# KyanChen/RSPrompter

Measured on NVIDIA H100. Metric: images/sec, higher is better.
Workload: dtype bf16

## Files before the change

### include/rsp_b200.h

```cpp
#ifndef RSP_B200_H_
#define RSP_B200_H_

#include <stdint.h>

#ifdef __cplusplus
extern "C" {
#endif

#define RSP_ABI_VERSION 2

int rsp_abi_version(void);
const char* rsp_last_error(void);

int rsp_gemm_bf16(const void* A, int lda, const void* W, int ldw, void* out, int ldo, int M, int N,
                  int K, const float* bias, const void* residual, int ldr, int res_fp32, int res_mod,
                  const int32_t* row_map, int act, int out_fp32, void* stream);

int rsp_conv3x3_nhwc_bf16(const void* x, int B, int H, int W, int C, const void* Wt, int ldw, void* out, int ldo,
                          int N, const float* bias, const void* residual, int ldr, int res_fp32, int act,
                          int out_fp32, void* stream);
int rsp_conv3x3_geometry_ok(int B, int H, int W, int C);

int rsp_gemm_bf16_simt(const void* A, int lda, const void* W, int ldw, void* out, int ldo, int M,
                       int N, int K, const float* bias, const void* residual, int ldr, int res_fp32,
                       int res_mod, const int32_t* row_map, int act, int out_fp32, void* stream);

int rsp_vit_attention(const void* qkv, const void* rel_h, const void* rel_w, void* out, int n_seq,
                      int T, int S, int H, int hd, void* stream);
int rsp_vit_attention_scatter(const void* qkv, const void* rel_h, const void* rel_w, void* out, int n_seq, int T,
                              int Sg, int H, int hd, const int32_t* out_row_map, void* stream);

int rsp_vit_attention_simt(const void* qkv, const void* rel_h, const void* rel_w, void* out,
                           int n_seq, int T, int S, int H, int hd, void* stream);

int rsp_layernorm(const void* in, int in_fp32, int ld_in, void* out, int out_fp32, int ld_out,
                  const float* gamma, const float* beta, const int32_t* src_map, int rows_out, int C,
                  float eps, int act, void* copy_out, int ld_copy, void* stream);

int rsp_layernorm_add(const void* x, const void* res, int res_fp32, const int32_t* res_block_map,
                      int res_block_rows, const float* gamma, const float* beta, void* out, const float* pos,
                      int pos_mod, void* out_pe, long long rows, int C, float eps, void* stream);

int rsp_patchify16(const float* img, void* out, int B, int H, int W, void* stream);

int rsp_im2col_nhwc(const void* in, void* out, int B, int H, int W, int C, int KH, int KW,
                    int stride, int pad, void* stream);

int rsp_nhwc_to_nchw(const void* in, int in_fp32, float* out, int B, int HW, int C, void* stream);

int rsp_gemm_bf16_ex(const void* A, int lda, const void* W, int ldw, void* out, int ldo, int M, int N,
                     int K, const float* bias, const void* residual, int ldr, int res_fp32, int res_mod,
                     const int32_t* row_map, int act, int out_fp32, int epi_mode, const float* ln_gamma,
                     const float* ln_beta, float ln_eps, const int32_t* res_block_map,
// ... 158 lines not shown
                         int64_t* offsets, void* stream);
int rsp_mask_rle_write(const uint8_t* src, int packed, const int64_t* desc, int n, const int64_t* offsets, char* pool,
                       int32_t* lengths, void* stream);
int rsp_mask_rle_placed_lengths(const uint8_t* src, int packed, const int64_t* desc, const int64_t* desc_host, int n,
                                int64_t* offsets, void* stream);
int rsp_mask_rle_placed_write(const uint8_t* src, int packed, const int64_t* desc, int n, const int64_t* offsets,
                              char* pool, int32_t* lengths, void* stream);


int rsp_preprocess_u8(const uint8_t* img, int h, int w, long long stride_c, long long stride_y, long long stride_x,
                      float* out, int H, int W, const float* mean3, const float* std3, int swap_rb, float pad_value,
                      void* stream);

int rsp_resize_pad_u8(const int64_t* desc, const int64_t* desc_host, int B, float* out, int Hp, int Wp,
                      const float* mean3, const float* std3, int swap_rb, const float* pad3, void* stream);

int rsp_patchify16_u8(const uint8_t* img, int hwc, void* out, int B, int H, int W, const float* mean3, const float* std3,
                      int swap_rb, void* stream);

int rsp_cast_f32_bf16(const float* in, void* out, long long n, void* stream);

int rsp_add_table_bf16(const void* x, const float* table, void* out, long long n, long long period, void* stream);

#ifdef __cplusplus
}
#endif
#endif
```

### rsprompter_b200/_lib.py

```python
from __future__ import annotations

import ctypes
import os
import subprocess
from pathlib import Path

import torch

_PKG_DIR = Path(__file__).resolve().parent
LIB_PATH = _PKG_DIR / "librsp_b200.so"
CSRC_DIR = _PKG_DIR / "csrc"


class RspError(RuntimeError):
    """Raised when an ``rsp_*`` entry point returns a non-zero status."""


def build_library(verbose: bool = False) -> Path:
    cmd = ["make", "-C", str(CSRC_DIR), "-j", str(os.cpu_count() or 4), "all"]
    res = subprocess.run(cmd, capture_output=True, text=True)
    if res.returncode != 0:
        raise RuntimeError(f"building librsp_b200.so failed:\n{res.stdout[-4000:]}\n{res.stderr[-4000:]}")
    if verbose:
        print(res.stdout[-2000:])
    return LIB_PATH


def _load() -> ctypes.CDLL:
    if not LIB_PATH.exists():
        raise ImportError(
            f"{LIB_PATH} not found: the CUDA extension is mandatory (no fallback path). "
            "Run `python -c 'import __graft_entry__ as g; g.build()'` or `make -C rsprompter_b200/csrc`.")
    return ctypes.CDLL(str(LIB_PATH))


_lib = _load()

_vp, _i, _f = ctypes.c_void_p, ctypes.c_int, ctypes.c_float

_SIGNATURES = {
    "rsp_abi_version": ([], _i),
    "rsp_last_error": ([], ctypes.c_char_p),
    "rsp_gemm_bf16": ([_vp, _i, _vp, _i, _vp, _i, _i, _i, _i, _vp, _vp, _i, _i, _i, _vp, _i, _i, _vp], _i),
    "rsp_gemm_bf16_simt": ([_vp, _i, _vp, _i, _vp, _i, _i, _i, _i, _vp, _vp, _i, _i, _i, _vp, _i, _i, _vp], _i),
    "rsp_vit_attention": ([_vp, _vp, _vp, _vp, _i, _i, _i, _i, _i, _vp], _i),
    "rsp_vit_attention_scatter": ([_vp, _vp, _vp, _vp, _i, _i, _i, _i, _i, _vp, _vp], _i),
    "rsp_vit_attention_simt": ([_vp, _vp, _vp, _vp, _i, _i, _i, _i, _i, _vp], _i),
    "rsp_layernorm": ([_vp, _i, _i, _vp, _i, _i, _vp, _vp, _vp, _i, _i, _f, _i, _vp, _i, _vp], _i),
    "rsp_patchify16": ([_vp, _vp, _i, _i, _i, _vp], _i),
    "rsp_layernorm_add": ([_vp, _vp, _i, _vp, _i, _vp, _vp, _vp, _vp, _i, _vp, ctypes.c_longlong, _i, _f, _vp], _i),
    "rsp_im2col_nhwc": ([_vp, _vp, _i, _i, _i, _i, _i, _i, _i, _i, _vp], _i),
    "rsp_nhwc_to_nchw": ([_vp, _i, _vp, _i, _i, _i, _vp], _i),
    "rsp_cast_f32_bf16": ([_vp, _vp, ctypes.c_longlong, _vp], _i),
    "rsp_add_table_bf16": ([_vp, _vp, _vp, ctypes.c_longlong, ctypes.c_longlong, _vp], _i),
    "rsp_gemm_bf16_ex": ([_vp, _i, _vp, _i, _vp, _i, _i, _i, _i, _vp, _vp, _i, _i, _i, _vp, _i, _i,
                          _i, _vp, _vp, _f, _vp, _i, _vp, _vp, _i, _i, _vp], _i),
    "rsp_add_cast_bf16": ([_vp, _vp, _vp, ctypes.c_longlong, ctypes.c_longlong, _vp], _i),
    "rsp_token_self_attention": ([_vp, _vp, _vp, _vp, _i, _i, _i, _i, _vp], _i),
    "rsp_t2i_attention": ([_vp, _vp, _vp, _i, _vp, _vp, _i, _i, _i, _vp], _i),
    "rsp_i2t_attention": ([_vp, _vp, _vp, _vp, _vp, _i, _i, _i, _vp], _i),
    "rsp_t2i_fused": ([_vp, _i, _vp, _vp, _vp, _vp, _vp, _i, _i, _i, _vp], _i),
    "rsp_i2t_fused": ([_vp, _i, _vp, _vp, _vp, _vp, _vp, _vp, _vp, _vp, _vp, _f, _vp, _i, _i, _i, _vp], _i),
    "rsp_rpn_decode": ([_vp, _i, _vp, _i, _i, _i, _i, _i, _i, _vp, _vp, _f, _f, _f, _i, _i, _vp, _vp, _vp], _i),
    "rsp_bbox_cls_decode": ([_vp, _i, _vp, _i, _vp, _vp, _i, _i, _vp, _f, _f, _f, _vp, _vp, _vp, _vp], _i),
    "rsp_rpn_decode_shapes": ([_vp, _i, _vp, _i, _i, _i, _i, _i, _i, _vp, _vp, _vp, _f, _i, _i, _vp, _vp, _vp], _i),
    "rsp_nms_batched_topk": ([_vp, _vp, _vp, _i, _i, _f, _vp, _vp, _vp, _i, _vp], _i),
    "rsp_bbox_cls_decode_shapes": ([_vp, _i, _vp, _i, _vp, _vp, _i, _i, _vp, _vp, _f, _vp, _vp, _vp, _vp], _i),
    "rsp_nms_batched": ([_vp, _vp, _vp, _i, _i, _f, _vp, _vp, _vp, _vp], _i),
    "rsp_compact_keep": ([_vp, _vp, _vp, _vp, _i, _i, _i, _vp, _vp, _vp, _vp, _vp, _vp], _i),
    "rsp_soft_nms_workspace_bytes": ([_i, _i, _i, _vp], _i),
    "rsp_soft_nms_batched": ([_vp, _vp, _vp, _vp, _i, _i, _i, _f, _f, _f, _i, _i, _i, _vp, ctypes.c_size_t, _vp, _vp,
                              _vp, _vp, _vp, _vp], _i),
    "rsp_roi_align_nhwc": ([_vp, _vp, _vp, _vp, _vp, _i, _vp, _i, _i, _i, _f, _vp, _vp], _i),
    "rsp_mask_paste": ([_vp, _vp, _i, _i, _i, _i, _i, _f, _i, _vp], _i),
    "rsp_pool2_nhwc": ([_vp, _vp, _i, _i, _i, _i, _i, _vp], _i),
    "rsp_zero_border_nhwc": ([_vp, _i, _i, _i, _i, _vp], _i),
    "rsp_sigmoid_f32": ([_vp, _vp, ctypes.c_longlong, _vp], _i),
# ... 336 lines not shown


def i2t_attention(Q: torch.Tensor, ktok: torch.Tensor, vtok: torch.Tensor, hw: int,
                  q_block: torch.Tensor | None = None) -> torch.Tensor:
    global launch_count
    _require_cuda(Q, ktok, vtok, q_block)
    N, Tq, C = ktok.shape
    assert C == 128 and Q.dtype == torch.bfloat16 and Q.is_contiguous() and Q.shape[1] == 128
    assert ktok.dtype == torch.bfloat16 and vtok.dtype == torch.bfloat16
    assert ktok.is_contiguous() and vtok.is_contiguous() and vtok.shape == ktok.shape
    if q_block is not None:
        assert q_block.dtype == torch.int32 and q_block.numel() == N and q_block.is_contiguous()
    else:
        assert Q.shape[0] == N * hw
    out = torch.empty((N * hw, 128), device=Q.device, dtype=torch.bfloat16)
    _check(_lib.rsp_i2t_attention(_ptr(Q), _ptr(q_block), _ptr(ktok), _ptr(vtok), _ptr(out), N, Tq, hw, _stream()),
           "rsp_i2t_attention")
    launch_count += 1
    return out


def vit_attention(qkv: torch.Tensor, rel_h: torch.Tensor, rel_w: torch.Tensor, n_seq: int, S: int,
                  H: int, hd: int, *, out: torch.Tensor | None = None, simt: bool = False,
                  out_row_map: torch.Tensor | None = None, out_rows: int | None = None) -> torch.Tensor:
    global launch_count
    _require_cuda(qkv, rel_h, rel_w, out)
    T = S * S
    D = H * hd
    if not simt and out_row_map is None and S not in (14, 32, 64) and T % 128 == 0 and S % 4 == 0:
        return vit_attention_generic(qkv, rel_h, rel_w, n_seq, S, H, hd, out=out)
    if not simt and S in (14, 32, 64):
        _log("attention_window" if S == 14 else "attention_global", 4.0 * n_seq * H * T * T * hd)
    assert qkv.dtype == torch.bfloat16 and qkv.is_contiguous() and qkv.shape == (n_seq * T, 3 * D)
    assert rel_h.dtype == torch.bfloat16 and rel_h.is_contiguous() and rel_h.shape == (2 * S - 1, hd)
    assert rel_w.dtype == torch.bfloat16 and rel_w.is_contiguous() and rel_w.shape == (2 * S - 1, hd)
    if out_row_map is not None:
        assert not simt and out_row_map.dtype == torch.int32 and out_row_map.is_contiguous()
        assert out_row_map.numel() == n_seq * T and out_rows is not None
        _require_cuda(out_row_map)
        if out is None:
            out = torch.empty((out_rows, D), device=qkv.device, dtype=torch.bfloat16)
        assert out.dtype == torch.bfloat16 and out.is_contiguous() and out.shape == (out_rows, D)
        _check(_lib.rsp_vit_attention_scatter(_ptr(qkv), _ptr(rel_h), _ptr(rel_w), _ptr(out), n_seq, T, S, H, hd,
                                              _ptr(out_row_map), _stream()), "rsp_vit_attention_scatter")
        launch_count += 1
        return out
    if out is None:
        out = torch.empty((n_seq * T, D), device=qkv.device, dtype=torch.bfloat16)
    assert out.dtype == torch.bfloat16 and out.is_contiguous() and out.shape == (n_seq * T, D)
    fn = _lib.rsp_vit_attention_simt if simt else _lib.rsp_vit_attention
    _check(fn(_ptr(qkv), _ptr(rel_h), _ptr(rel_w), _ptr(out), n_seq, T, S, H, hd, _stream()),
           "rsp_vit_attention")
    launch_count += 1
    return out


def gemm_grouped(a: torch.Tensor, w: torch.Tensor, out: torch.Tensor, N: int, m_group_rows: int, w_group_rows: int,
                 row_map: torch.Tensor | None = None) -> torch.Tensor:
    global launch_count
    _require_cuda(a, w, out, row_map)
    assert a.dtype == torch.bfloat16 and w.dtype == torch.bfloat16 and a.dim() == 2 and w.dim() == 2
    assert a.stride(1) == 1 and w.stride(1) == 1 and out.dim() == 2 and out.stride(1) == 1
    M, K = a.shape
    assert w.shape[1] == K and M % m_group_rows == 0 and m_group_rows % 128 == 0
    assert w.shape[0] >= (M // m_group_rows - 1) * w_group_rows + N and out.shape[1] >= N
    assert out.dtype in (torch.bfloat16, torch.float32)
    if row_map is not None:
        assert row_map.dtype == torch.int32 and row_map.numel() == M and row_map.is_contiguous()
    _check(_lib.rsp_gemm_bf16_grouped(_ptr(a), a.stride(0), _ptr(w), w.stride(0), _ptr(out), out.stride(0), M, N, K,
                                      m_group_rows, w_group_rows, _ptr(row_map), int(out.dtype == torch.float32),
                                      _stream()), "rsp_gemm_bf16_grouped")
    launch_count += 1
    _log("gemm", 2.0 * M * N * K)
    return out

# ... 835 lines not shown
```

### rsprompter_b200/csrc/abi.cu

```cuda
#include "../../include/rsp_b200.h"

#include "attention.h"
#include "gemm.h"
#include "rowops.h"

namespace rsp { const char* last_error(); }
using namespace rsp;

static inline cudaStream_t S(void* s) { return static_cast<cudaStream_t>(s); }

extern "C" {

int rsp_abi_version(void) { return RSP_ABI_VERSION; }
const char* rsp_last_error(void) { return rsp::last_error(); }

static GemmArgs make_gemm_args(const void* A, int lda, const void* W, int ldw, void* out, int ldo,
                               int M, int N, int K, const float* bias, const void* residual, int ldr,
                               int res_fp32, int res_mod, const int32_t* row_map, int act,
                               int out_fp32) {
  GemmArgs a;
  a.A = A; a.lda = lda; a.W = W; a.ldw = ldw; a.out = out; a.ldo = ldo;
  a.M = M; a.N = N; a.K = K; a.bias = bias; a.residual = residual; a.ldr = ldr;
  a.res_fp32 = res_fp32; a.res_mod = res_mod; a.row_map = row_map; a.act = act;
  a.out_fp32 = out_fp32;
// ... 30 lines not shown
                       int res_mod, const int32_t* row_map, int act, int out_fp32, void* stream) {
  return gemm_bf16_simt(make_gemm_args(A, lda, W, ldw, out, ldo, M, N, K, bias, residual, ldr,
                                       res_fp32, res_mod, row_map, act, out_fp32), S(stream));
}

static AttentionArgs make_att_args(const void* qkv, const void* rel_h, const void* rel_w, void* out,
                                   int n_seq, int T, int Sg, int H, int hd, const int32_t* out_row_map = nullptr) {
  AttentionArgs a;
  a.qkv = qkv; a.rel_h = rel_h; a.rel_w = rel_w; a.out = out;
  a.n_seq = n_seq; a.T = T; a.S = Sg; a.H = H; a.hd = hd; a.out_row_map = out_row_map;
  return a;
}

int rsp_vit_attention(const void* qkv, const void* rel_h, const void* rel_w, void* out, int n_seq,
                      int T, int Sg, int H, int hd, void* stream) {
  return vit_attention(make_att_args(qkv, rel_h, rel_w, out, n_seq, T, Sg, H, hd), S(stream));
}

int rsp_vit_attention_scatter(const void* qkv, const void* rel_h, const void* rel_w, void* out, int n_seq, int T,
                              int Sg, int H, int hd, const int32_t* out_row_map, void* stream) {
  return vit_attention(make_att_args(qkv, rel_h, rel_w, out, n_seq, T, Sg, H, hd, out_row_map), S(stream));
}

int rsp_vit_attention_simt(const void* qkv, const void* rel_h, const void* rel_w, void* out,
                           int n_seq, int T, int Sg, int H, int hd, void* stream) {
  return vit_attention_simt(make_att_args(qkv, rel_h, rel_w, out, n_seq, T, Sg, H, hd), S(stream));
}

int rsp_attn_softmax_bias(const float* scores, int lds, const float* tab, int ldt, int NT, void* P, int ldp, int n_rows,
                          int T, int Sg, float scale, void* stream) {
  return attn_softmax_bias(scores, lds, tab, ldt, NT, P, ldp, n_rows, T, Sg, scale, S(stream));
}

int rsp_transpose_cols(const void* in, int ld, int col0, int C, int n_seq, int T, void* out, void* stream) {
  return transpose_cols(in, ld, col0, C, n_seq, T, out, S(stream));
}

int rsp_split_heads(const void* in, int ld, int col0, int H, int hd, int n_seq, int T, void* out, void* stream) {
  return split_heads(in, ld, col0, H, hd, n_seq, T, out, S(stream));
}

int rsp_layernorm(const void* in, int in_fp32, int ld_in, void* out, int out_fp32, int ld_out,
                  const float* gamma, const float* beta, const int32_t* src_map, int rows_out, int C,
                  float eps, int act, void* copy_out, int ld_copy, void* stream) {
  LayerNormArgs a;
  a.copy_out = copy_out; a.ld_copy = ld_copy;
// ... 9 lines not shown
  return layernorm_add(x, res, res_fp32, res_block_map, res_block_rows, gamma, beta, out, pos, pos_mod, out_pe, rows,
                       C, eps, S(stream));
}

int rsp_patchify16(const float* img, void* out, int B, int H, int W, void* stream) {
  return patchify16(img, out, B, H, W, S(stream));
}

int rsp_im2col_nhwc(const void* in, void* out, int B, int H, int W, int C, int KH, int KW,
                    int stride, int pad, void* stream) {
  return im2col_nhwc(in, out, B, H, W, C, KH, KW, stride, pad, S(stream));
}

int rsp_nhwc_to_nchw(const void* in, int in_fp32, float* out, int B, int HW, int C, void* stream) {
  return nhwc_to_nchw(in, in_fp32, out, B, HW, C, S(stream));
}

int rsp_cast_f32_bf16(const float* in, void* out, long long n, void* stream) {
  return cast_f32_bf16(in, out, n, S(stream));
}

int rsp_add_table_bf16(const void* x, const float* table, void* out, long long n, long long period, void* stream) {
  return add_table_bf16(x, table, out, n, period, S(stream));
}

}

#include "decoder.h"

extern "C" {

int rsp_gemm_bf16_ex(const void* A, int lda, const void* W, int ldw, void* out, int ldo, int M, int N,
                     int K, const float* bias, const void* residual, int ldr, int res_fp32, int res_mod,
                     const int32_t* row_map, int act, int out_fp32, int epi_mode, const float* ln_gamma,
                     const float* ln_beta, float ln_eps, const int32_t* res_block_map,
                     int res_block_rows, const float* hyper, float* mask_out, int grid_h, int grid_w,
                     void* stream) {
  GemmArgs a = make_gemm_args(A, lda, W, ldw, out, ldo, M, N, K, bias, residual, ldr, res_fp32,
                              res_mod, row_map, act, out_fp32);
  a.epi_mode = epi_mode; a.ln_gamma = ln_gamma; a.ln_beta = ln_beta; a.ln_eps = ln_eps;
  a.res_block_map = res_block_map; a.res_block_rows = res_block_rows;
  a.hyper = hyper; a.mask_out = mask_out; a.grid_h = grid_h; a.grid_w = grid_w;
  return gemm_bf16(a, S(stream));
}

int rsp_gemm_upscale_masks(const void* A, int lda, const void* W, int ldw, int M, int K, const float* bias,
// ... 341 lines not shown
```

### rsprompter_b200/csrc/attention.cu

```cuda
#include <cstdlib>

#include "attention.h"
#include "sm90.cuh"

namespace rsp {

constexpr float LOG2E = 1.4426950408889634f;

__device__ __forceinline__ float fast_exp2(float x) {
  float y;
  asm("ex2.approx.ftz.f32 %0, %1;" : "=f"(y) : "f"(x));
  return y;
}
__device__ __forceinline__ uint32_t pack_f16x2(float lo, float hi) {
  __half2 v = __floats2half2_rn(lo, hi);
  return *reinterpret_cast<uint32_t*>(&v);
}
__device__ __forceinline__ uint32_t bf16x2_to_f16x2(uint32_t w) {
  return pack_f16x2(__uint_as_float(w << 16), __uint_as_float(w & 0xffff0000u));
}

template <int HD, int S>
struct AttCfg {
  static constexpr int T = S * S;
// ... 7 lines not shown
  static constexpr int STAGES = 4;
  static constexpr int SP = S + 4;
  __host__ __device__ static constexpr int tile_bytes(int rows) { return rows * (128 + 2 * TAIL); }
  static constexpr int STAGE_BYTES = 2 * tile_bytes(BN);
  static constexpr int smem_bytes(int qbuf) {
    return qbuf * tile_bytes(BM) + STAGES * STAGE_BYTES + 2 * tile_bytes(NTAB) + 2 * BM * SP * 4 + 8 * 64 + 1024;
  }
  static constexpr int QBUF = smem_bytes(2) <= 227 * 1024 ? 2 : 1;
  static constexpr int Q_OFF = 0;
  static constexpr int KV_OFF = Q_OFF + QBUF * tile_bytes(BM);
  static constexpr int TAB_OFF = KV_OFF + STAGES * STAGE_BYTES;
  static constexpr int BIAS_OFF = TAB_OFF + 2 * tile_bytes(NTAB);
  static constexpr int BAR_OFF = BIAS_OFF + 2 * BM * SP * 4;
  static constexpr int SMEM_BYTES = smem_bytes(QBUF);
  static constexpr int REG_PRODUCER = 40, REG_CONSUMER = 232;
  static_assert(HD == 64 || HD == 80, "head dim");
  static_assert(NREL <= 128, "table rows");
  static_assert(SMEM_BYTES <= 227 * 1024, "shared memory");
};

struct AttDev {
  __nv_bfloat16* out;
  const int* out_row_map;
  int H;
  int D;
  int n_items;
  float scale2;
};

template <int N, int TAIL>
__device__ __forceinline__ void qk_wgmma(float (&acc)[N / 2], uint32_t qa, uint32_t qtail, uint32_t b, int b_rows) {
  acc_fence(acc);
  wgmma_fence();
#pragma unroll
  for (int k = 0; k < 4; ++k)
    Wgmma<N>::template ss<0>(acc, make_gdesc(qa + 32 * k, 16, 1024), make_gdesc(b + 32 * k, 16, 1024), k);
  if constexpr (TAIL > 0)
    Wgmma<N>::template ss<0>(acc, make_gdesc_sw32(qtail, 16, 256), make_gdesc_sw32(b + b_rows * 128, 16, 256), 1);
  wgmma_commit();
  wgmma_wait<0>();
  acc_fence(acc);
}

template <int TAIL>
__device__ __forceinline__ void load_tile(uint32_t dst, int rows, const CUtensorMap* m, const CUtensorMap* mt,
                                          uint32_t bar, int col, int row, int seq) {
// ... 6 lines not shown
vit_attention_kernel(const __grid_constant__ CUtensorMap tm_q, const __grid_constant__ CUtensorMap tm_q_t,
                     const __grid_constant__ CUtensorMap tm_kv, const __grid_constant__ CUtensorMap tm_kv_t,
                     const __grid_constant__ CUtensorMap tm_rh, const __grid_constant__ CUtensorMap tm_rh_t,
                     const __grid_constant__ CUtensorMap tm_rw, const __grid_constant__ CUtensorMap tm_rw_t,
                     const AttDev p) {
  using C = AttCfg<HD, S>;
  constexpr int T = C::T, BM = C::BM, BN = C::BN, NKT = C::NKT, SP = C::SP, STAGES = C::STAGES, TAIL = C::TAIL;
  constexpr int QBUF = C::QBUF;
  constexpr uint32_t TILE_KV = C::tile_bytes(BN), TILE_TAB = C::tile_bytes(C::NTAB);
  extern __shared__ __align__(1024) uint8_t smem_raw[];
  uint8_t* smem = smem_raw + ((1024u - (smem_u32(smem_raw) & 1023u)) & 1023u);
  const uint32_t sbase = smem_u32(smem);
  float* relh = reinterpret_cast<float*>(smem + C::BIAS_OFF);
  float* relw = relh + BM * SP;
  uint64_t* bar_tab = reinterpret_cast<uint64_t*>(smem + C::BAR_OFF);
  uint64_t* bar_q = bar_tab + 1;
  uint64_t* bar_qe = bar_q + QBUF;
  uint64_t* bar_k = bar_qe + QBUF;
  uint64_t* bar_v = bar_k + STAGES;
  uint64_t* bar_vc = bar_v + STAGES;
  uint64_t* bar_e = bar_vc + STAGES;

  const int warp = threadIdx.x >> 5, lane = threadIdx.x & 31;
  auto decode = [&](int item, int& q0, int& head, int& seq) {
    q0 = (item % C::NQT) * BM;
    item /= C::NQT;
    head = item % p.H;
    seq = item / p.H;
  };

  if (threadIdx.x == 0) {
    tma_prefetch_desc(&tm_q);
    tma_prefetch_desc(&tm_kv);
    mbar_init(smem_u32(bar_tab), 1);
    for (int b = 0; b < QBUF; ++b) {
      mbar_init(smem_u32(&bar_q[b]), 1);
      mbar_init(smem_u32(&bar_qe[b]), 8);
    }
    for (int s = 0; s < STAGES; ++s) {
      mbar_init(smem_u32(&bar_k[s]), 1);
      mbar_init(smem_u32(&bar_v[s]), 1);
      mbar_init(smem_u32(&bar_vc[s]), 3);
      mbar_init(smem_u32(&bar_e[s]), 8);
    }
    fence_barrier_init();
  }
  __syncthreads();
// ... 239 lines not shown
  const uint32_t qbox[3] = {64, C::BM, 1}, qbox_t[3] = {16, C::BM, 1};
  const uint32_t kvbox[3] = {64, C::BN, 1}, kvbox_t[3] = {16, C::BN, 1};
  const uint32_t tbox[2] = {64, static_cast<uint32_t>(C::NTAB)}, tbox_t[2] = {16, static_cast<uint32_t>(C::NTAB)};
  CUtensorMap tq, tkv, th, tw, tq_t, tkv_t, th_t, tw_t;
  RSP_TRY(make_tmap_swizzled(&tq, a.qkv, 3, qdims, qstr, qbox, 0, 128));
  RSP_TRY(make_tmap_swizzled(&tkv, a.qkv, 3, qdims, qstr, kvbox, 0, 128));
  RSP_TRY(make_tmap_swizzled(&th, a.rel_h, 2, tdims, tstr, tbox, 0, 128));
  RSP_TRY(make_tmap_swizzled(&tw, a.rel_w, 2, tdims, tstr, tbox, 0, 128));
  if (C::TAIL > 0) {
    RSP_TRY(make_tmap_swizzled(&tq_t, a.qkv, 3, qdims, qstr, qbox_t, 0, 32));
    RSP_TRY(make_tmap_swizzled(&tkv_t, a.qkv, 3, qdims, qstr, kvbox_t, 0, 32));
    RSP_TRY(make_tmap_swizzled(&th_t, a.rel_h, 2, tdims, tstr, tbox_t, 0, 32));
    RSP_TRY(make_tmap_swizzled(&tw_t, a.rel_w, 2, tdims, tstr, tbox_t, 0, 32));
  } else {
    tq_t = tq; tkv_t = tkv; th_t = th; tw_t = tw;
  }
  auto kern = vit_attention_kernel<HD, S>;
  static bool attr_set_dev[kMaxDevices] = {};
  bool& attr_set = attr_set_dev[current_device()];
  if (!attr_set) {
    RSP_CHECK_CUDA(cudaFuncSetAttribute(kern, cudaFuncAttributeMaxDynamicSharedMemorySize, C::SMEM_BYTES));
    attr_set = true;
  }
  const long long items = static_cast<long long>(a.n_seq) * a.H * C::NQT;
  RSP_CHECK_ARG(items > 0 && items < (1ll << 31), "attention: %lld query tiles", items);
  p.n_items = static_cast<int>(items);
  const int grid = static_cast<int>(items < num_sms() ? items : num_sms());
  kern<<<grid, 384, C::SMEM_BYTES, stream>>>(tq, tq_t, tkv, tkv_t, th, th_t, tw, tw_t, p);
  RSP_CHECK_LAUNCH();
  return RSP_OK;
}

int vit_attention(const AttentionArgs& a, cudaStream_t stream) {
  RSP_CHECK_ARG(a.qkv && a.rel_h && a.rel_w && a.out, "attention: null pointer");
  RSP_CHECK_ARG(a.T == a.S * a.S, "attention: T=%d is not S^2 (S=%d)", a.T, a.S);
  RSP_CHECK_ARG(a.n_seq > 0 && a.H > 0, "attention: bad n_seq/H");
  if (a.S != 14 && a.S != 32 && a.S != 64)
    return vit_attention_simt(a, stream);
  if (a.hd == 64) {
    if (a.S == 64) return launch_att<64, 64>(a, stream);
    if (a.S == 32) return launch_att<64, 32>(a, stream);
    return launch_att<64, 14>(a, stream);
  }
  if (a.hd == 80) {
    if (a.S == 64) return launch_att<80, 64>(a, stream);
    if (a.S == 32) return launch_att<80, 32>(a, stream);
    return launch_att<80, 14>(a, stream);
  }
// ... 66 lines not shown
```

### rsprompter_b200/csrc/attention.h

```cpp
#pragma once
#include "host_util.h"

namespace rsp {

struct AttentionArgs {
  const void* qkv = nullptr;
  const void* rel_h = nullptr;
  const void* rel_w = nullptr;
  void* out = nullptr;
  int n_seq = 0;
  int T = 0;
  int S = 0;
  int H = 0;
  int hd = 0;
  const int* out_row_map = nullptr;
};

int vit_attention(const AttentionArgs& a, cudaStream_t stream);
int vit_attention_simt(const AttentionArgs& a, cudaStream_t stream);
int attn_softmax_bias(const float* scores, int lds, const float* tab, int ldt, int NT, void* P, int ldp, int n_rows,
                      int T, int S, float scale, cudaStream_t stream);
int transpose_cols(const void* in, int ld, int col0, int C, int n_seq, int T, void* out, cudaStream_t stream);
int split_heads(const void* in, int ld, int col0, int H, int hd, int n_seq, int T, void* out, cudaStream_t stream);

}
```

### rsprompter_b200/csrc/rowops.cu

```cuda
#include "rowops.h"
#include "sm90.cuh"

namespace rsp {

template <typename T>
__device__ __forceinline__ float load_as_float(const T* p);
template <>
__device__ __forceinline__ float load_as_float<float>(const float* p) { return *p; }
template <>
__device__ __forceinline__ float load_as_float<__nv_bfloat16>(const __nv_bfloat16* p) {
  return __bfloat162float(*p);
}

template <typename TIn, typename TOut, int MAXV>
__global__ void layernorm_rows_kernel(const TIn* __restrict__ in, TOut* __restrict__ out,
                                      const float* __restrict__ gamma,
                                      const float* __restrict__ beta,
                                      const int* __restrict__ src_map, int rows_out, int C,
                                      int ld_in, int ld_out, float eps, int act,
                                      __nv_bfloat16* __restrict__ copy_out, int ld_copy) {
  const int warps_per_block = blockDim.x >> 5;
  const int row = blockIdx.x * warps_per_block + (threadIdx.x >> 5);
  const int lane = threadIdx.x & 31;
  if (row >= rows_out) return;
// ... 328 lines not shown
  const long long i = static_cast<long long>(blockIdx.x) * blockDim.x + threadIdx.x;
  if (i >= n8) return;
  const uint4 u = x[i];
  const float* t = table + (i * 8) % period;
  const float4 t0 = *reinterpret_cast<const float4*>(t), t1 = *reinterpret_cast<const float4*>(t + 4);
  const uint32_t w[4] = {u.x, u.y, u.z, u.w};
  const float tv[8] = {t0.x, t0.y, t0.z, t0.w, t1.x, t1.y, t1.z, t1.w};
  uint32_t o[4];
#pragma unroll
  for (int j = 0; j < 4; ++j)
    o[j] = pack_bf16x2(__uint_as_float(w[j] << 16) + tv[2 * j], __uint_as_float(w[j] & 0xffff0000u) + tv[2 * j + 1]);
  out[i] = make_uint4(o[0], o[1], o[2], o[3]);
}

int add_table_bf16(const void* x, const float* table, void* out, long long n, long long period, cudaStream_t stream) {
  RSP_CHECK_ARG(x && table && out && n > 0 && n % 8 == 0 && period > 0 && period % 8 == 0, "add_table: bad args");
  const long long n8 = n / 8;
  add_table_bf16_kernel<<<static_cast<unsigned>((n8 + 255) / 256), 256, 0, stream>>>(
      static_cast<const uint4*>(x), table, static_cast<uint4*>(out), n8, period);
  RSP_CHECK_LAUNCH();
  return RSP_OK;
}

}
```

### rsprompter_b200/csrc/rowops.h

```cpp
#pragma once
#include "host_util.h"

namespace rsp {

struct LayerNormArgs {
  const void* in = nullptr;
  void* out = nullptr;
  const float* gamma = nullptr;
  const float* beta = nullptr;
  const int* src_map = nullptr;
  int rows_out = 0, C = 0, ld_in = 0, ld_out = 0;
  float eps = 1e-6f;
  int act = 0;
  int in_fp32 = 1, out_fp32 = 0;
  void* copy_out = nullptr;
  int ld_copy = 0;
};

int layernorm_rows(const LayerNormArgs& a, cudaStream_t stream);
int patchify16(const float* img, void* out, int B, int Himg, int Wimg, cudaStream_t stream);
int im2col_nhwc(const void* in, void* out, int B, int H, int W, int C, int KH, int KW, int stride,
                int pad, cudaStream_t stream);
int nhwc_to_nchw(const void* in, int in_fp32, float* out, int B, int HW, int C, cudaStream_t stream);

int layernorm_add(const void* x, const void* res, int res_fp32, const int* res_block_map, int res_block_rows,
                  const float* gamma, const float* beta, void* out, const float* pos, int pos_mod, void* out_pe,
                  long long rows, int C, float eps, cudaStream_t stream);
int cast_f32_bf16(const float* in, void* out, long long n, cudaStream_t stream);
int add_table_bf16(const void* x, const float* table, void* out, long long n, long long period, cudaStream_t stream);

}
```

### rsprompter_b200/sam_encoder.py

```python
from __future__ import annotations

import re
from collections import OrderedDict

import torch
from torch import nn

from . import _lib
from .registry import MODELS, BaseModule
from .sam_config import SamVisionArch, parse_arch_name, vision_arch

try:
    from transformers.models.sam.modeling_sam import SamVisionEncoderOutput as _HFOut
except Exception:
    _HFOut = None


if _HFOut is not None:
    SamVisionEncoderOutput = _HFOut
else:
    class SamVisionEncoderOutput(tuple):

        def __new__(cls, last_hidden_state=None, hidden_states=None, **_):
            items = tuple(x for x in (last_hidden_state, hidden_states) if x is not None)
# ... 45 lines not shown
        super().__init__()
        self.projection = _Affine((D, 3, p, p))


class _Neck(nn.Module):
    def __init__(self, D: int, C: int):
        super().__init__()
        self.conv1 = _Affine((C, D, 1, 1), bias=False)
        self.layer_norm1 = _Affine((C,))
        self.conv2 = _Affine((C, C, 3, 3), bias=False)
        self.layer_norm2 = _Affine((C,))


def window_maps(batch: int, grid: int, window: int, device: torch.device) -> tuple[torch.Tensor, int]:
    nw = (grid + window - 1) // window
    gp = nw * window
    ys = torch.arange(gp, device=device)
    tok = ys[:, None] * grid + ys[None, :]
    tok = torch.where((ys[:, None] < grid) & (ys[None, :] < grid), tok, torch.full_like(tok, -1))
    tok = tok.reshape(nw, window, nw, window).permute(0, 2, 1, 3).reshape(-1)
    off = (torch.arange(batch, device=device) * grid * grid)[:, None]
    full = torch.where(tok[None, :] >= 0, tok[None, :] + off, torch.full_like(tok[None, :], -1))
    return full.reshape(-1).to(torch.int32).contiguous(), nw * nw


class SamVisionEncoderB200(nn.Module):

    def __init__(self, arch: SamVisionArch):
        super().__init__()
        self.arch = arch
        D, g = arch.hidden_size, arch.grid
        self.patch_embed = _PatchEmbed(D, arch.patch_size)
        self.pos_embed = nn.Parameter(torch.empty(1, g, g, D), requires_grad=False)
        self.layers = nn.ModuleList(
            _Layer(arch, g if i in arch.global_attn_indexes else arch.window_size)
            for i in range(arch.num_layers))
        self.neck = _Neck(D, arch.output_channels)
        self._prep: dict | None = None
        self._maps: dict = {}
        self.register_load_state_dict_post_hook(lambda *_: self._invalidate())
        self._register_load_state_dict_pre_hook(self._resize_checkpoint_tables)

    def _resize_checkpoint_tables(self, state_dict, prefix, *args):
        import torch.nn.functional as F
        k = prefix + "pos_embed"
        if k in state_dict and tuple(state_dict[k].shape) != tuple(self.pos_embed.shape):
# ... 29 lines not shown
        D, C = a.hidden_size, a.output_channels
        p: dict = {}
        p["pe_w"] = bf(self.patch_embed.projection.weight.reshape(D, -1))
        p["pe_b"] = f32(self.patch_embed.projection.bias)
        p["pos"] = f32(self.pos_embed.reshape(-1, D))
        layers = []
        for lyr in self.layers:
            layers.append(dict(
                ln1_w=f32(lyr.layer_norm1.weight), ln1_b=f32(lyr.layer_norm1.bias),
                ln2_w=f32(lyr.layer_norm2.weight), ln2_b=f32(lyr.layer_norm2.bias),
                qkv_w=bf(lyr.attn.qkv.weight), qkv_b=f32(lyr.attn.qkv.bias),
                proj_w=bf(lyr.attn.proj.weight), proj_b=f32(lyr.attn.proj.bias),
                rel_h=bf(lyr.attn.rel_pos_h), rel_w=bf(lyr.attn.rel_pos_w),
                lin1_w=bf(lyr.mlp.lin1.weight), lin1_b=f32(lyr.mlp.lin1.bias),
                lin2_w=bf(lyr.mlp.lin2.weight), lin2_b=f32(lyr.mlp.lin2.bias)))
        p["layers"] = layers
        p["n1_w"] = bf(self.neck.conv1.weight.reshape(C, D))
        p["n2_w"] = bf(self.neck.conv2.weight.permute(0, 2, 3, 1).reshape(C, 9 * C))
        p["nln1_w"], p["nln1_b"] = f32(self.neck.layer_norm1.weight), f32(self.neck.layer_norm1.bias)
        p["nln2_w"], p["nln2_b"] = f32(self.neck.layer_norm2.weight), f32(self.neck.layer_norm2.bias)
        self._prep = p
        return p

    def _window_map(self, batch: int, device: torch.device) -> tuple[torch.Tensor, int]:
        key = (batch, device)
        if key not in self._maps:
            self._maps[key] = window_maps(batch, self.arch.grid, self.arch.window_size, device)
        return self._maps[key]

    @torch.no_grad()
    def encode(self, pixel_values: torch.Tensor, want_hidden: bool = True, bf16_copies: dict | None = None):
        a = self.arch
        if pixel_values.dim() != 4 or pixel_values.shape[1] != 3:
            raise ValueError("Make sure that the channel dimension of the pixel values match with the "
                             "one set in the configuration.")
        B, _, Hi, Wi = pixel_values.shape
        if Hi != a.image_size or Wi != a.image_size:
            raise ValueError(f"Input image size ({Hi}*{Wi}) doesn't match model ({a.image_size}*{a.image_size}).")
        p = self._prep or self._prepare()
        D, g, H, hd, C = a.hidden_size, a.grid, a.num_heads, a.head_dim, a.output_channels
        T = g * g
        M = B * T
        if pixel_values.dtype == torch.uint8:
            norm = getattr(pixel_values, "rsp_norm", None)
            if norm is None:
                raise _lib.RspError("uint8 pixel_values need the DetDataPreprocessor normalisation (tensor.rsp_norm)")
            x = pixel_values
            patches = _lib.patchify16_u8(x, norm[0], norm[1], norm[2])
        else:
            x = pixel_values.to(dtype=torch.float32).contiguous()
            patches = _lib.patchify16(x)
        h = _lib.gemm(patches, p["pe_w"], p["pe_b"], residual=p["pos"], res_mod=T,
                      out_dtype=torch.float32)
        hidden = [h]
        wmap, n_win = self._window_map(B, x.device)
        ws = a.window_size
        for i, lw in enumerate(p["layers"]):
            is_global = i in a.global_attn_indexes
            cp = None
            if bf16_copies is not None and i in bf16_copies:
                cp = torch.empty(M, D, device=x.device, dtype=torch.bfloat16)
                bf16_copies[i] = cp.view(B, g, g, D)
            if is_global:
                xn = _lib.layernorm(h, lw["ln1_w"], lw["ln1_b"], a.layer_norm_eps, copy_out=cp)
                qkv = _lib.gemm(xn, lw["qkv_w"], lw["qkv_b"])
                att = _lib.vit_attention(qkv, lw["rel_h"], lw["rel_w"], B, g, H, hd)
                x1 = _lib.gemm(att, lw["proj_w"], lw["proj_b"], residual=h, out_dtype=torch.float32)
            else:
                xn = _lib.layernorm(h, lw["ln1_w"], lw["ln1_b"], a.layer_norm_eps, src_map=wmap, copy_out=cp)
                qkv = _lib.gemm(xn, lw["qkv_w"], lw["qkv_b"])
                att = _lib.vit_attention(qkv, lw["rel_h"], lw["rel_w"], B * n_win, ws, H, hd, out_row_map=wmap,
                                         out_rows=M)
                x1 = _lib.gemm(att, lw["proj_w"], lw["proj_b"], residual=h, out_dtype=torch.float32)
            xn2 = _lib.layernorm(x1, lw["ln2_w"], lw["ln2_b"], a.layer_norm_eps)
            y = _lib.gemm(xn2, lw["lin1_w"], lw["lin1_b"], act="gelu")
            h = _lib.gemm(y, lw["lin2_w"], lw["lin2_b"], residual=x1, out_dtype=torch.float32)
            hidden.append(h)
        hb = _lib.cast_bf16(h)
        c1 = _lib.gemm(hb, p["n1_w"])
        l1 = _lib.layernorm(c1, p["nln1_w"], p["nln1_b"], 1e-6)
        if _lib.conv3x3_ok(B, g, g, C):
            c2 = _lib.conv3x3_nhwc(l1.view(B, g, g, C), p["n2_w"])
        else:
            c2 = _lib.gemm(_lib.im2col_nhwc(l1.view(B, g, g, C), 3, 3, 1, 1), p["n2_w"])
        l2 = _lib.layernorm(c2, p["nln2_w"], p["nln2_b"], 1e-6, out_dtype=torch.float32)
        emb = _lib.nhwc_to_nchw(l2.view(B, g, g, C))
        hs = tuple(t.view(B, g, g, D) for t in hidden) if want_hidden else None
        return emb, hs, l2.view(B, g, g, C)

    def forward(self, pixel_values: torch.Tensor | None = None, **kwargs):
        if pixel_values is None:
            raise ValueError("You have to specify pixel_values")
        emb, hs, _ = self.encode(pixel_values, want_hidden=self.arch.output_hidden_states)
        return SamVisionEncoderOutput(last_hidden_state=emb, hidden_states=hs)


# ... 107 lines not shown
    def _rename_mmpretrain_keys(state_dict, prefix, *args):
        pre = prefix + "vision_encoder."
        for k in [k for k in state_dict if k.startswith(pre)]:
            k2 = k[len(pre):]
            for pat, rep in _MMPRETRAIN_TO_HF:
                k2 = re.sub(pat, rep, k2)
            if pre + k2 != k:
                state_dict[pre + k2] = state_dict.pop(k)

    def load_mmpretrain_state_dict(self, sd: dict) -> None:
        out = OrderedDict()
        for k, v in sd.items():
            for pat, rep in _MMPRETRAIN_TO_HF:
                k = re.sub(pat, rep, k)
            out[k] = v
        self.vision_encoder.load_state_dict(out)

    def forward(self, x):
        emb, _, _ = self.vision_encoder.encode(x, want_hidden=False)
        return (emb,)


__all__ = ["SamVisionEncoderB200", "RSSamVisionEncoder", "MMPretrainSamVisionEncoder",
           "SamVisionEncoderOutput", "window_maps", "parse_arch_name"]
```

Before: 63.13.

## Skip padded window rows in QKV GEMM and attention query tiles

Windowed layers previously ran the QKV GEMM over the padded window layout, including pad rows. Now the GEMM runs over the real tokens and scatters rows into the padded layout via an inverse row map, and a small kernel fills the pad rows with the bias. Attention is launched over a precomputed list of query tiles that contain at least one real token, so tiles made only of padding are skipped. This adds an extra kernel launch and indirection through a tile list, and relies on the GEMM's row-map scatter path being efficient.

After: 63.54, median of 6. About the same (+0.6%).

```diff
diff --git a/include/rsp_b200.h b/include/rsp_b200.h
--- a/include/rsp_b200.h
+++ b/include/rsp_b200.h
@@ -29,6 +29,9 @@
                       int T, int S, int H, int hd, void* stream);
 int rsp_vit_attention_scatter(const void* qkv, const void* rel_h, const void* rel_w, void* out, int n_seq, int T,
                               int Sg, int H, int hd, const int32_t* out_row_map, void* stream);
+int rsp_vit_attention_scatter_tiles(const void* qkv, const void* rel_h, const void* rel_w, void* out, int n_seq, int T,
+                                    int Sg, int H, int hd, const int32_t* out_row_map, const int32_t* tiles,
+                                    int n_tiles, void* stream);
 
 int rsp_vit_attention_simt(const void* qkv, const void* rel_h, const void* rel_w, void* out,
                            int n_seq, int T, int S, int H, int hd, void* stream);
@@ -233,6 +236,8 @@
 
 int rsp_add_table_bf16(const void* x, const float* table, void* out, long long n, long long period, void* stream);
 
+int rsp_fill_rows_bias(void* out, int ldo, const int32_t* rows, int n_rows, const float* bias, int N, void* stream);
+
 #ifdef __cplusplus
 }
 #endif
diff --git a/profiles/window_padding_bench.py b/profiles/window_padding_bench.py
--- /dev/null
+++ b/profiles/window_padding_bench.py
@@ -0,0 +1,82 @@
+import argparse
+import json
+import os
+import statistics
+import subprocess
+import sys
+
+ROOT = os.path.dirname(os.path.dirname(os.path.abspath(__file__)))
+if ROOT not in sys.path:
+    sys.path.insert(0, ROOT)
+
+import torch
+
+from rsprompter_b200 import _lib
+from rsprompter_b200.sam_encoder import window_layout
+
+
+def _time(fn, calls=20, reps=5):
+    for _ in range(3):
+        fn()
+    ms = []
+    for _ in range(reps):
+        a, b = torch.cuda.Event(enable_timing=True), torch.cuda.Event(enable_timing=True)
+        a.record()
+        for _ in range(calls):
+            fn()
+        b.record()
+        torch.cuda.synchronize()
+        ms.append(a.elapsed_time(b) / calls)
+    return statistics.median(ms)
+
+
+def main():
+    ap = argparse.ArgumentParser()
+    ap.add_argument("--sizes", type=int, nargs="+", default=[512, 768, 1024])
+    ap.add_argument("--batch", type=int, default=8)
+    args = ap.parse_args()
+    card = subprocess.run(["nvidia-smi", "--query-gpu=name,power.limit,clocks.max.sm", "--format=csv,noheader"],
+                          capture_output=True, text=True).stdout.strip()
+    D, H, hd, B = 1280, 16, 80, args.batch
+    g = torch.Generator().manual_seed(0)
+    w = (torch.randn(3 * D, D, generator=g) * D ** -0.5).to(torch.bfloat16).cuda()
+    bias = torch.randn(3 * D, generator=g).cuda()
+    ln_w, ln_b = torch.ones(D, device="cuda"), torch.zeros(D, device="cuda")
+    rh = (torch.randn(27, hd, generator=g) * 0.2).to(torch.bfloat16).cuda()
+    rw = (torch.randn(27, hd, generator=g) * 0.2).to(torch.bfloat16).cuda()
+    for size in args.sizes:
+        grid = size // 16
+        M = B * grid * grid
+        wl = window_layout(B, grid, 14, H, torch.device("cuda"))
+        n_seq = B * wl["n_win"]
+        h = torch.randn(M, D, generator=g).cuda()
+
+        def qkv_old():
+            return _lib.gemm(_lib.layernorm(h, ln_w, ln_b, 1e-6, src_map=wl["map"]), w, bias)
+
+        def qkv_new():
+            q = _lib.gemm(_lib.layernorm(h, ln_w, ln_b, 1e-6), w, bias, row_map=wl["inv"], out_rows=wl["map"].numel())
+            return _lib.fill_rows_bias(q, wl["pad"], bias)
+
+        qkv = qkv_old()
+        assert torch.equal(qkv.view(torch.int16), qkv_new().view(torch.int16))
+        xn = _lib.layernorm(h, ln_w, ln_b, 1e-6)
+        xn_pad = _lib.layernorm(h, ln_w, ln_b, 1e-6, src_map=wl["map"])
+        q_out = torch.empty_like(qkv)
+        res = dict(card=card, size=size, batch=B, real_rows=M, padded_rows=wl["map"].numel(),
+                   tiles=wl["tiles"].numel(), all_tiles=n_seq * H * 2)
+        res["qkv_old_ms"] = _time(qkv_old)
+        res["qkv_new_ms"] = _time(qkv_new)
+        res["gemm_padded_ms"] = _time(lambda: _lib.gemm(xn_pad, w, bias, out=q_out))
+        res["gemm_rowmap_ms"] = _time(lambda: _lib.gemm(xn, w, bias, row_map=wl["inv"], out=q_out))
+        res["fill_pad_ms"] = _time(lambda: _lib.fill_rows_bias(q_out, wl["pad"], bias))
+        att = torch.empty(M, D, device="cuda", dtype=torch.bfloat16)
+        res["attn_all_ms"] = _time(lambda: _lib.vit_attention(qkv, rh, rw, n_seq, 14, H, hd, out=att,
+                                                              out_row_map=wl["map"], out_rows=M))
+        res["attn_tiles_ms"] = _time(lambda: _lib.vit_attention(qkv, rh, rw, n_seq, 14, H, hd, out=att,
+                                                                out_row_map=wl["map"], out_rows=M, tiles=wl["tiles"]))
+        print(json.dumps({k: round(v, 4) if isinstance(v, float) else v for k, v in res.items()}), flush=True)
+
+
+if __name__ == "__main__":
+    main()
diff --git a/rsprompter_b200/_lib.py b/rsprompter_b200/_lib.py
--- a/rsprompter_b200/_lib.py
+++ b/rsprompter_b200/_lib.py
@@ -45,6 +45,7 @@
     "rsp_gemm_bf16_simt": ([_vp, _i, _vp, _i, _vp, _i, _i, _i, _i, _vp, _vp, _i, _i, _i, _vp, _i, _i, _vp], _i),
     "rsp_vit_attention": ([_vp, _vp, _vp, _vp, _i, _i, _i, _i, _i, _vp], _i),
     "rsp_vit_attention_scatter": ([_vp, _vp, _vp, _vp, _i, _i, _i, _i, _i, _vp, _vp], _i),
+    "rsp_vit_attention_scatter_tiles": ([_vp, _vp, _vp, _vp, _i, _i, _i, _i, _i, _vp, _vp, _i, _vp], _i),
     "rsp_vit_attention_simt": ([_vp, _vp, _vp, _vp, _i, _i, _i, _i, _i, _vp], _i),
     "rsp_layernorm": ([_vp, _i, _i, _vp, _i, _i, _vp, _vp, _vp, _i, _i, _f, _i, _vp, _i, _vp], _i),
     "rsp_patchify16": ([_vp, _vp, _i, _i, _i, _vp], _i),
@@ -53,6 +54,7 @@
     "rsp_nhwc_to_nchw": ([_vp, _i, _vp, _i, _i, _i, _vp], _i),
     "rsp_cast_f32_bf16": ([_vp, _vp, ctypes.c_longlong, _vp], _i),
     "rsp_add_table_bf16": ([_vp, _vp, _vp, ctypes.c_longlong, ctypes.c_longlong, _vp], _i),
+    "rsp_fill_rows_bias": ([_vp, _i, _vp, _i, _vp, _i, _vp], _i),
     "rsp_gemm_bf16_ex": ([_vp, _i, _vp, _i, _vp, _i, _i, _i, _i, _vp, _vp, _i, _i, _i, _vp, _i, _i,
                           _i, _vp, _vp, _f, _vp, _i, _vp, _vp, _i, _i, _vp], _i),
     "rsp_add_cast_bf16": ([_vp, _vp, _vp, ctypes.c_longlong, ctypes.c_longlong, _vp], _i),
@@ -435,7 +437,8 @@
 
 def vit_attention(qkv: torch.Tensor, rel_h: torch.Tensor, rel_w: torch.Tensor, n_seq: int, S: int,
                   H: int, hd: int, *, out: torch.Tensor | None = None, simt: bool = False,
-                  out_row_map: torch.Tensor | None = None, out_rows: int | None = None) -> torch.Tensor:
+                  out_row_map: torch.Tensor | None = None, out_rows: int | None = None,
+                  tiles: torch.Tensor | None = None) -> torch.Tensor:
     global launch_count
     _require_cuda(qkv, rel_h, rel_w, out)
     T = S * S
@@ -454,16 +457,36 @@
         if out is None:
             out = torch.empty((out_rows, D), device=qkv.device, dtype=torch.bfloat16)
         assert out.dtype == torch.bfloat16 and out.is_contiguous() and out.shape == (out_rows, D)
-        _check(_lib.rsp_vit_attention_scatter(_ptr(qkv), _ptr(rel_h), _ptr(rel_w), _ptr(out), n_seq, T, S, H, hd,
-                                              _ptr(out_row_map), _stream()), "rsp_vit_attention_scatter")
+        if tiles is not None:
+            assert tiles.dtype == torch.int32 and tiles.is_contiguous() and tiles.dim() == 1
+            _require_cuda(tiles)
+            _check(_lib.rsp_vit_attention_scatter_tiles(_ptr(qkv), _ptr(rel_h), _ptr(rel_w), _ptr(out), n_seq, T, S,
+                                                        H, hd, _ptr(out_row_map), _ptr(tiles), tiles.numel(),
+                                                        _stream()), "rsp_vit_attention_scatter_tiles")
+        else:
+            _check(_lib.rsp_vit_attention_scatter(_ptr(qkv), _ptr(rel_h), _ptr(rel_w), _ptr(out), n_seq, T, S, H, hd,
+                                                  _ptr(out_row_map), _stream()), "rsp_vit_attention_scatter")
         launch_count += 1
         return out
     if out is None:
         out = torch.empty((n_seq * T, D), device=qkv.device, dtype=torch.bfloat16)
     assert out.dtype == torch.bfloat16 and out.is_contiguous() and out.shape == (n_seq * T, D)
+    assert tiles is None, "a query-tile list goes with out_row_map"
     fn = _lib.rsp_vit_attention_simt if simt else _lib.rsp_vit_attention
     _check(fn(_ptr(qkv), _ptr(rel_h), _ptr(rel_w), _ptr(out), n_seq, T, S, H, hd, _stream()),
            "rsp_vit_attention")
+    launch_count += 1
+    return out
+
+
+def fill_rows_bias(out: torch.Tensor, rows: torch.Tensor, bias: torch.Tensor) -> torch.Tensor:
+    global launch_count
+    _require_cuda(out, rows, bias)
+    assert out.dtype == torch.bfloat16 and out.dim() == 2 and out.stride(1) == 1
+    assert rows.dtype == torch.int32 and rows.is_contiguous() and rows.dim() == 1
+    assert bias.dtype == torch.float32 and bias.is_contiguous() and bias.numel() == out.shape[1]
+    _check(_lib.rsp_fill_rows_bias(_ptr(out), out.stride(0), _ptr(rows), rows.numel(), _ptr(bias), out.shape[1],
+                                   _stream()), "rsp_fill_rows_bias")
     launch_count += 1
     return out
 
diff --git a/rsprompter_b200/csrc/abi.cu b/rsprompter_b200/csrc/abi.cu
--- a/rsprompter_b200/csrc/abi.cu
+++ b/rsprompter_b200/csrc/abi.cu
@@ -76,6 +76,20 @@
   return vit_attention(make_att_args(qkv, rel_h, rel_w, out, n_seq, T, Sg, H, hd, out_row_map), S(stream));
 }
 
+int rsp_vit_attention_scatter_tiles(const void* qkv, const void* rel_h, const void* rel_w, void* out, int n_seq, int T,
+                                    int Sg, int H, int hd, const int32_t* out_row_map, const int32_t* tiles,
+                                    int n_tiles, void* stream) {
+  if (Sg != 14 && Sg != 32 && Sg != 64) {
+    set_last_error("attention: a query-tile list needs the tensor-core kernel (S = 14, 32 or 64), not S = %d", Sg);
+    return RSP_ERR_UNSUPPORTED;
+  }
+  AttentionArgs a = make_att_args(qkv, rel_h, rel_w, out, n_seq, T, Sg, H, hd, out_row_map);
+  RSP_CHECK_ARG(tiles != nullptr, "attention: null query-tile list");
+  a.items = tiles;
+  a.n_items = n_tiles;
+  return vit_attention(a, S(stream));
+}
+
 int rsp_vit_attention_simt(const void* qkv, const void* rel_h, const void* rel_w, void* out,
                            int n_seq, int T, int Sg, int H, int hd, void* stream) {
   return vit_attention_simt(make_att_args(qkv, rel_h, rel_w, out, n_seq, T, Sg, H, hd), S(stream));
@@ -131,6 +145,10 @@
 
 int rsp_add_table_bf16(const void* x, const float* table, void* out, long long n, long long period, void* stream) {
   return add_table_bf16(x, table, out, n, period, S(stream));
+}
+
+int rsp_fill_rows_bias(void* out, int ldo, const int32_t* rows, int n_rows, const float* bias, int N, void* stream) {
+  return fill_rows_bias(out, ldo, rows, n_rows, bias, N, S(stream));
 }
 
 }
diff --git a/rsprompter_b200/csrc/attention.cu b/rsprompter_b200/csrc/attention.cu
--- a/rsprompter_b200/csrc/attention.cu
+++ b/rsprompter_b200/csrc/attention.cu
@@ -53,6 +53,7 @@
 struct AttDev {
   __nv_bfloat16* out;
   const int* out_row_map;
+  const int* items;
   int H;
   int D;
   int n_items;
@@ -105,7 +106,8 @@
   uint64_t* bar_e = bar_vc + STAGES;
 
   const int warp = threadIdx.x >> 5, lane = threadIdx.x & 31;
-  auto decode = [&](int item, int& q0, int& head, int& seq) {
+  auto decode = [&](int i, int& q0, int& head, int& seq) {
+    int item = p.items ? __ldg(p.items + i) : i;
     q0 = (item % C::NQT) * BM;
     item /= C::NQT;
     head = item % p.H;
@@ -391,8 +393,13 @@
     RSP_CHECK_CUDA(cudaFuncSetAttribute(kern, cudaFuncAttributeMaxDynamicSharedMemorySize, C::SMEM_BYTES));
     attr_set = true;
   }
-  const long long items = static_cast<long long>(a.n_seq) * a.H * C::NQT;
+  long long items = static_cast<long long>(a.n_seq) * a.H * C::NQT;
   RSP_CHECK_ARG(items > 0 && items < (1ll << 31), "attention: %lld query tiles", items);
+  p.items = a.items;
+  if (a.items) {
+    RSP_CHECK_ARG(a.n_items > 0 && a.n_items <= items, "attention: %d listed query tiles of %lld", a.n_items, items);
+    items = a.n_items;
+  }
   p.n_items = static_cast<int>(items);
   const int grid = static_cast<int>(items < num_sms() ? items : num_sms());
   kern<<<grid, 384, C::SMEM_BYTES, stream>>>(tq, tq_t, tkv, tkv_t, th, th_t, tw, tw_t, p);
diff --git a/rsprompter_b200/csrc/attention.h b/rsprompter_b200/csrc/attention.h
--- a/rsprompter_b200/csrc/attention.h
+++ b/rsprompter_b200/csrc/attention.h
@@ -14,6 +14,8 @@
   int H = 0;
   int hd = 0;
   const int* out_row_map = nullptr;
+  const int* items = nullptr;
+  int n_items = 0;
 };
 
 int vit_attention(const AttentionArgs& a, cudaStream_t stream);
diff --git a/rsprompter_b200/csrc/rowops.cu b/rsprompter_b200/csrc/rowops.cu
--- a/rsprompter_b200/csrc/rowops.cu
+++ b/rsprompter_b200/csrc/rowops.cu
@@ -374,4 +374,29 @@
   return RSP_OK;
 }
 
-}
+__global__ void fill_rows_bias_kernel(uint4* __restrict__ out, long long ldo8, const int* __restrict__ rows,
+                                      const float* __restrict__ bias, int n8) {
+  uint4* o = out + static_cast<long long>(__ldg(rows + blockIdx.x)) * ldo8;
+  for (int j = threadIdx.x; j < n8; j += blockDim.x) {
+    const float4 b0 = __ldg(reinterpret_cast<const float4*>(bias) + 2 * j);
+    const float4 b1 = __ldg(reinterpret_cast<const float4*>(bias) + 2 * j + 1);
+    o[j] = make_uint4(pack_bf16x2(__fadd_rn(0.f, b0.x), __fadd_rn(0.f, b0.y)),
+                      pack_bf16x2(__fadd_rn(0.f, b0.z), __fadd_rn(0.f, b0.w)),
+                      pack_bf16x2(__fadd_rn(0.f, b1.x), __fadd_rn(0.f, b1.y)),
+                      pack_bf16x2(__fadd_rn(0.f, b1.z), __fadd_rn(0.f, b1.w)));
+  }
+}
+
+int fill_rows_bias(void* out, int ldo, const int* rows, int n_rows, const float* bias, int N, cudaStream_t stream) {
+  RSP_CHECK_ARG(out && rows && bias && n_rows >= 0 && N > 0 && N % 8 == 0 && ldo % 8 == 0 && ldo >= N &&
+                    (reinterpret_cast<uintptr_t>(out) & 15) == 0 && (reinterpret_cast<uintptr_t>(bias) & 15) == 0,
+                "fill_rows_bias: bad args");
+  if (n_rows == 0) return RSP_OK;
+  const int n8 = N / 8;
+  fill_rows_bias_kernel<<<n_rows, n8 < 512 ? ((n8 + 31) / 32) * 32 : 512, 0, stream>>>(
+      static_cast<uint4*>(out), ldo / 8, rows, bias, n8);
+  RSP_CHECK_LAUNCH();
+  return RSP_OK;
+}
+
+}
diff --git a/rsprompter_b200/csrc/rowops.h b/rsprompter_b200/csrc/rowops.h
--- a/rsprompter_b200/csrc/rowops.h
+++ b/rsprompter_b200/csrc/rowops.h
@@ -28,5 +28,6 @@
                   long long rows, int C, float eps, cudaStream_t stream);
 int cast_f32_bf16(const float* in, void* out, long long n, cudaStream_t stream);
 int add_table_bf16(const void* x, const float* table, void* out, long long n, long long period, cudaStream_t stream);
+int fill_rows_bias(void* out, int ldo, const int* rows, int n_rows, const float* bias, int N, cudaStream_t stream);
 
 }
diff --git a/rsprompter_b200/sam_encoder.py b/rsprompter_b200/sam_encoder.py
--- a/rsprompter_b200/sam_encoder.py
+++ b/rsprompter_b200/sam_encoder.py
@@ -91,6 +91,23 @@
     off = (torch.arange(batch, device=device) * grid * grid)[:, None]
     full = torch.where(tok[None, :] >= 0, tok[None, :] + off, torch.full_like(tok[None, :], -1))
     return full.reshape(-1).to(torch.int32).contiguous(), nw * nw
+
+
+def window_layout(batch: int, grid: int, window: int, heads: int, device: torch.device) -> dict:
+    wmap, n_win = window_maps(batch, grid, window, torch.device("cpu"))
+    T = window * window
+    real = wmap >= 0
+    inv = torch.empty(batch * grid * grid, dtype=torch.int32)
+    inv[wmap[real].long()] = torch.arange(wmap.numel(), dtype=torch.int32)[real]
+    pad = torch.nonzero(~real).flatten().to(torch.int32)
+    tiles = None
+    if window in (14, 32, 64):
+        nqt = (T + 127) // 128
+        r = torch.zeros(batch * n_win, nqt * 128, dtype=torch.bool)
+        r[:, :T] = real.view(batch * n_win, T)
+        keep = r.view(batch * n_win, 1, nqt, 128).any(-1).expand(batch * n_win, heads, nqt).reshape(-1)
+        tiles = torch.nonzero(keep).flatten().to(torch.int32).to(device)
+    return dict(map=wmap.to(device), n_win=n_win, inv=inv.to(device), pad=pad.to(device), tiles=tiles)
 
 
 class SamVisionEncoderB200(nn.Module):
@@ -166,10 +183,11 @@
         self._prep = p
         return p
 
-    def _window_map(self, batch: int, device: torch.device) -> tuple[torch.Tensor, int]:
+    def _window_layout(self, batch: int, device: torch.device) -> dict:
         key = (batch, device)
         if key not in self._maps:
-            self._maps[key] = window_maps(batch, self.arch.grid, self.arch.window_size, device)
+            a = self.arch
+            self._maps[key] = window_layout(batch, a.grid, a.window_size, a.num_heads, device)
         return self._maps[key]
 
     @torch.no_grad()
@@ -197,7 +215,7 @@
         h = _lib.gemm(patches, p["pe_w"], p["pe_b"], residual=p["pos"], res_mod=T,
                       out_dtype=torch.float32)
         hidden = [h]
-        wmap, n_win = self._window_map(B, x.device)
+        wl = self._window_layout(B, x.device)
         ws = a.window_size
         for i, lw in enumerate(p["layers"]):
             is_global = i in a.global_attn_indexes
@@ -205,17 +223,16 @@
             if bf16_copies is not None and i in bf16_copies:
                 cp = torch.empty(M, D, device=x.device, dtype=torch.bfloat16)
                 bf16_copies[i] = cp.view(B, g, g, D)
+            xn = _lib.layernorm(h, lw["ln1_w"], lw["ln1_b"], a.layer_norm_eps, copy_out=cp)
             if is_global:
-                xn = _lib.layernorm(h, lw["ln1_w"], lw["ln1_b"], a.layer_norm_eps, copy_out=cp)
                 qkv = _lib.gemm(xn, lw["qkv_w"], lw["qkv_b"])
                 att = _lib.vit_attention(qkv, lw["rel_h"], lw["rel_w"], B, g, H, hd)
-                x1 = _lib.gemm(att, lw["proj_w"], lw["proj_b"], residual=h, out_dtype=torch.float32)
             else:
-                xn = _lib.layernorm(h, lw["ln1_w"], lw["ln1_b"], a.layer_norm_eps, src_map=wmap, copy_out=cp)
-                qkv = _lib.gemm(xn, lw["qkv_w"], lw["qkv_b"])
-                att = _lib.vit_attention(qkv, lw["rel_h"], lw["rel_w"], B * n_win, ws, H, hd, out_row_map=wmap,
-                                         out_rows=M)
-                x1 = _lib.gemm(att, lw["proj_w"], lw["proj_b"], residual=h, out_dtype=torch.float32)
+                qkv = _lib.gemm(xn, lw["qkv_w"], lw["qkv_b"], row_map=wl["inv"], out_rows=wl["map"].numel())
+                _lib.fill_rows_bias(qkv, wl["pad"], lw["qkv_b"])
+                att = _lib.vit_attention(qkv, lw["rel_h"], lw["rel_w"], B * wl["n_win"], ws, H, hd,
+                                         out_row_map=wl["map"], out_rows=M, tiles=wl["tiles"])
+            x1 = _lib.gemm(att, lw["proj_w"], lw["proj_b"], residual=h, out_dtype=torch.float32)
             xn2 = _lib.layernorm(x1, lw["ln2_w"], lw["ln2_b"], a.layer_norm_eps)
             y = _lib.gemm(xn2, lw["lin1_w"], lw["lin1_b"], act="gelu")
             h = _lib.gemm(y, lw["lin2_w"], lw["lin2_b"], residual=x1, out_dtype=torch.float32)
@@ -369,4 +386,4 @@
 
 
 __all__ = ["SamVisionEncoderB200", "RSSamVisionEncoder", "MMPretrainSamVisionEncoder",
-           "SamVisionEncoderOutput", "window_maps", "parse_arch_name"]
+           "SamVisionEncoderOutput", "window_maps", "window_layout", "parse_arch_name"]
```
